# ubuntuslave/vo_single_camera_sos

Hardware: AMD Instinct MI355X
Metric: frame-pairs/sec (detect+match+triangulate+RANSAC) on 640x480 omni, 2000 kpts (higher is better)
Workload: dtype u8/f32/f64

## Files before the change

vo_single_camera_sos_amd/csrc/ransac.hip:

```cpp
#include <type_traits>
#include "common.h"
#include "ransac_core.h"
#include "epnp_core.h"
#include "gp3p_core.h"

namespace {

constexpr int kMaxCam = 8;
constexpr int kHypDoubles = 16;
constexpr int kThreads = 256;
constexpr int kScoreHypChunkMax = 128;

__device__ const double kEye9[9] = {1, 0, 0, 0, 1, 0, 0, 0, 1};
__device__ const double kZero3[3] = {0, 0, 0};

__device__ __forceinline__ uint64_t problem_seed(uint64_t seed, int b) { return seed + (uint64_t)b; }
__device__ __forceinline__ uint64_t problem_seed(const uint64_t* seeds, int b) { return seeds[b]; }

__global__ __launch_bounds__(kThreads) void ransac_prepare_kernel(const int32_t* __restrict__ cam,
                                                                  const int32_t* __restrict__ n_arr, int stride,
                                                                  int ncam, int32_t* __restrict__ perm,
                                                                  int32_t* __restrict__ cinfo) {
  SOSVO_LATENCY_BOUND_PRIO();
  __shared__ int cnt[kThreads][kMaxCam];
// ... 116 lines not shown
  const int it = chunk * 64 + threadIdx.x;
  const int n = min(n_arr[b], stride);
  const size_t base = (size_t)b * stride;
  double R[9], t[3];
  int ok = 0;
  if (it < H) ok = sv_hypothesis_twopt(f + 3 * base, p + 3 * base, n, problem_seed(seed, b), (uint64_t)it, R, t);
  hyp_store_wave(hyp + (size_t)b * H * kHypDoubles, chunk * 64, H, ok != 0, R, t);
  if (it < H) counts[(size_t)b * H + it] = ok ? 0 : -1;
}

template <class SeedT>
__global__ __launch_bounds__(64) __attribute__((amdgpu_waves_per_eu(3, 3))) void ransac_hyp_gp3p_kernel(const double* __restrict__ f, const double* __restrict__ p,
                                                             const int32_t* __restrict__ cam,
                                                             const double* __restrict__ cam_off,
                                                             const double* __restrict__ cam_rot,
                                                             const int32_t* __restrict__ n_arr, int nprob, int stride,
                                                             int H, SeedT seed, double* __restrict__ hyp,
                                                             int32_t* __restrict__ counts) {
  SOSVO_LATENCY_BOUND_PRIO();
  int b, chunk;
  if (!hyp_block(nprob, (H + 63) >> 6, &b, &chunk)) return;
  const int it = chunk * 64 + threadIdx.x;
  const int n = min(n_arr[b], stride);
  const size_t base = (size_t)b * stride;
  const double* off = cam ? cam_off : kZero3;
  const double* rot = cam ? cam_rot : kEye9;
  double R[9], t[3];
  int ok = 0;
  if (it < H)
    ok = sv_hypothesis_gp3p(f + 3 * base, p + 3 * base, cam ? cam + base : nullptr, off, rot, n, problem_seed(seed, b),
                            (uint64_t)it, R, t);
  hyp_store_wave(hyp + (size_t)b * H * kHypDoubles, chunk * 64, H, ok != 0, R, t);
  if (it < H) counts[(size_t)b * H + it] = ok ? 0 : -1;
}

__device__ __forceinline__ int epnp_sample_front(const double* __restrict__ f, const double* __restrict__ p, int n, size_t base,
                                                 uint64_t seed, int it, double (&p6)[18], double (&uv)[2 * SV_EPNP_MAXN],
                                                 double (&cw)[12], double (&alphas)[4 * SV_EPNP_MAXN]) {
  int32_t s6[6];
  if (!sv_sample_distinct(n, 6, seed, (uint64_t)it, s6)) return 0;
  double f6[18];
#pragma unroll
  for (int k = 0; k < 6; ++k)
#pragma unroll
    for (int c = 0; c < 3; ++c) {
      f6[3 * k + c] = f[3 * (base + s6[k]) + c];
      p6[3 * k + c] = p[3 * (base + s6[k]) + c];
    }
  return sv_epnp_front(f6, p6, 6, uv, cw, alphas);
}

constexpr int kEpnpVecDoubles = 48;
template <class SeedT>
__global__ __launch_bounds__(64) void ransac_epnp_eigen_kernel(const double* __restrict__ f, const double* __restrict__ p,
                                                               const int32_t* __restrict__ n_arr, int nprob, int stride,
                                                               int H, SeedT seed, double* __restrict__ vvbuf,
                                                               int32_t* __restrict__ counts) {
  int b, chunk;
  if (!hyp_block(nprob, (H + 63) >> 6, &b, &chunk)) return;
  const int it = chunk * 64 + threadIdx.x;
  if (it >= H) return;
  const int n = min(n_arr[b], stride);
  double p6[18], uv[2 * SV_EPNP_MAXN], cw[12], alphas[4 * SV_EPNP_MAXN];
  int ok = epnp_sample_front(f, p, n, (size_t)b * stride, problem_seed(seed, b), it, p6, uv, cw, alphas);
  double* out = vvbuf + ((size_t)b * H + it) * kEpnpVecDoubles;
  if (ok) {
    double vv[48];
    ok = sv_epnp_null4_ql(alphas, uv, 6, vv);
    if (ok) {
#pragma unroll
      for (int k = 0; k < 48; ++k) out[k] = vv[k];
    }
  }
  counts[(size_t)b * H + it] = ok ? 0 : -1;
}

template <class SeedT>
__global__ __launch_bounds__(64) void ransac_epnp_pose_kernel(const double* __restrict__ f, const double* __restrict__ p,
                                                              const int32_t* __restrict__ n_arr, int nprob, int stride,
                                                              int H, SeedT seed, const double* __restrict__ vvbuf,
                                                              double* __restrict__ hyp, int32_t* __restrict__ counts) {
  SOSVO_LATENCY_BOUND_PRIO();
  int b, chunk;
  if (!hyp_block(nprob, (H + 63) >> 6, &b, &chunk)) return;
  const int it = chunk * 64 + threadIdx.x;
  const int n = min(n_arr[b], stride);
  double R[9], t[3];
  int ok = it < H && counts[(size_t)b * H + it] == 0;
  if (ok) {
    double p6[18], uv[2 * SV_EPNP_MAXN], cw[12], alphas[4 * SV_EPNP_MAXN], vv[48];
    ok = epnp_sample_front(f, p, n, (size_t)b * stride, problem_seed(seed, b), it, p6, uv, cw, alphas);
    const double* in = vvbuf + ((size_t)b * H + it) * kEpnpVecDoubles;
#pragma unroll
    for (int k = 0; k < 48; ++k) vv[k] = in[k];
    if (ok) ok = sv_epnp_back(p6, 6, uv, cw, alphas, vv, R, t);
  }
  hyp_store_wave(hyp + (size_t)b * H * kHypDoubles, chunk * 64, H, ok != 0, R, t);
  if (it < H) counts[(size_t)b * H + it] = ok ? 0 : -1;
}

template <bool IDENT>
__device__ __forceinline__ bool inlier_exact(const double* __restrict__ h, const double fx, const double fy,
                                             const double fz, const double px, const double py, const double pz,
                                             const double ox, const double oy, const double oz, const double* Rc,
                                             const double thr) {
  const double vx = (((h[0] * px) + (h[3] * py)) + (h[6] * pz)) + h[12];
  const double vy = (((h[1] * px) + (h[4] * py)) + (h[7] * pz)) + h[13];
  const double vz = (((h[2] * px) + (h[5] * py)) + (h[8] * pz)) + h[14];
  const double wx = vx - ox, wy = vy - oy, wz = vz - oz;
  double ux = wx, uy = wy, uz = wz;
  if (!IDENT) {
    ux = ((Rc[0] * wx) + (Rc[3] * wy)) + (Rc[6] * wz);
    uy = ((Rc[1] * wx) + (Rc[4] * wy)) + (Rc[7] * wz);
    uz = ((Rc[2] * wx) + (Rc[5] * wy)) + (Rc[8] * wz);
  }
  const double nrm = sqrt(((ux * ux) + (uy * uy)) + (uz * uz));
  const double gx = ux / nrm, gy = uy / nrm, gz = uz / nrm;
  return (1.0 - (((fx * gx) + (fy * gy)) + (fz * gz))) < thr;
}

constexpr double kTier1K = 1048576.0;
constexpr double kTier1Eps = 5.9604644775390625e-08;
constexpr double kTier1QBand = 3.47 / kTier1K + 20.0 * kTier1Eps;
constexpr double kTier1Max = 1e9;
constexpr double kTier1E2 = (3.47 * kTier1K + 6.0) * 78.03 * kTier1Eps * kTier1Eps * (1.0 + 1e-4);

__device__ __forceinline__ float score_tier1_lane(double fx, double fy, double fz, double px, double py, double pz, double ox,
                                                  double oy, double oz) {
  const double p1 = fabs(px) + fabs(py) + fabs(pz);
  const double om = fmax(fabs(ox), fmax(fabs(oy), fabs(oz)));
  const double fn = fx * fx + fy * fy + fz * fz;
  const double l = (p1 * p1 + om * om) * (1.0 + 1e-6);
  return (fabs(fn - 1.0) <= 1e-6 && p1 <= kTier1Max && om <= kTier1Max) ? (float)l : __builtin_inff();
}

__device__ __forceinline__ void score_tier1_hyp(const double* __restrict__ h, float* __restrict__ hs) {
  double rho = 0.0;
#pragma unroll
  for (int k = 0; k < 9; ++k) {
    hs[k] = (float)h[k];
    rho = fmax(rho, fabs(h[k]));
  }
  const double im = fmax(fabs(h[9]), fmax(fabs(h[10]), fabs(h[11])));
  hs[9] = (float)h[9], hs[10] = (float)h[10], hs[11] = (float)h[11];
  const double chk = (((((((h[0] + h[1]) + h[2]) + h[3]) + h[4]) + h[5]) + h[6]) + h[7]) + h[8] + h[9] + h[10] + h[11];
  const double ea = kTier1E2 * fmax(rho * rho, 1.0) * (1.0 + 1e-6);
  const double eb = kTier1E2 * (im * im) * (1.0 + 1e-6) + 1e-24;
  const bool fin = chk == chk && rho <= kTier1Max && im <= kTier1Max;
  hs[12] = fin ? (float)ea : __builtin_nanf("");
  hs[13] = fin ? (float)eb : __builtin_nanf("");
  hs[14] = 0.0f, hs[15] = 0.0f;
}

template <bool IDENT, int PPT, bool T1>
__global__ __launch_bounds__(kThreads) __attribute__((amdgpu_waves_per_eu(T1 ? 4 : 1))) void ransac_score_kernel(
    const double* __restrict__ f, const double* __restrict__ p, const int32_t* __restrict__ cam,
    const double* __restrict__ cam_off, const double* __restrict__ cam_rot, const int32_t* __restrict__ n_arr,
    int stride, int H, int hchunk, int hspan, double thr, int fast_ok, const double* __restrict__ hyp,
    int32_t* __restrict__ counts, int set_lo, int set_hi, int hsplit, const int32_t* __restrict__ alive_idx,
    const int32_t* __restrict__ n_alive) {
  static_assert(!T1 || (IDENT && PPT <= 4), "tier 1 is written for the identity-rotation form");
  SOSVO_LATENCY_BOUND_PRIO();
  constexpr bool KEEP = !T1;
  __shared__ int lcnt[kScoreHypChunkMax];
  __shared__ double shyp[kScoreHypChunkMax][12];
  __shared__ unsigned long long sok[(kScoreHypChunkMax + 63) / 64];
  __shared__ int sidx[kScoreHypChunkMax];
  __shared__ int srec[kScoreHypChunkMax];
  __shared__ float shyp32[T1 ? kScoreHypChunkMax : 1][16];
  const int tid = threadIdx.x, b = blockIdx.z;
  const int n = min(n_arr[b], stride);
  const int Hb = alive_idx ? n_alive[b] : H;
  const int xspan = alive_idx ? (int)((blockIdx.x + blockIdx.z) % gridDim.x) : (int)blockIdx.x;
  if (xspan * hspan >= Hb) return;
  const int sbeg = set_lo, send = min((n + 63) >> 6, set_hi);
  const int nsets = send - sbeg;
  const int bcap = hsplit ? PPT : (kThreads / 64) * PPT;
  const int nb = (nsets + bcap - 1) / bcap;
  if ((int)blockIdx.y >= nb) return;
  const int spb = (nsets + nb - 1) / nb;
  const int set0 = hsplit ? sbeg + ((int)blockIdx.y * nsets) / nb : sbeg + (int)blockIdx.y * spb;
  const int set1 = hsplit ? sbeg + (((int)blockIdx.y + 1) * nsets) / nb : min(set0 + spb, send);
  const int p0 = set0 * 64;

  double fx[KEEP ? PPT : 1], fy[KEEP ? PPT : 1], fz[KEEP ? PPT : 1];
  double px[KEEP ? PPT : 1], py[KEEP ? PPT : 1], pz[KEEP ? PPT : 1];
  double ox[KEEP ? PPT : 1], oy[KEEP ? PPT : 1], oz[KEEP ? PPT : 1];
  float fxs[T1 ? PPT : 1], fys[T1 ? PPT : 1], fzs[T1 ? PPT : 1], pxs[T1 ? PPT : 1], pys[T1 ? PPT : 1], pzs[T1 ? PPT : 1];
  float oxs[T1 ? PPT : 1], oys[T1 ? PPT : 1], ozs[T1 ? PPT : 1], lerr[T1 ? PPT : 1];
  int rowi[PPT];
  double Rc[IDENT ? 1 : 9];
  const int wave = __builtin_amdgcn_readfirstlane(tid >> 6), lane = tid & 63;
  const int wslot = (wave + blockIdx.x + blockIdx.y + blockIdx.z) & (kThreads / 64 - 1);
  const int jstep = hsplit ? kThreads / 64 : 1, jbeg = hsplit ? wslot : 0;
  const size_t base = (size_t)b * stride;
  unsigned long long vmask[PPT];
  int nlive_v = 0;
#pragma unroll
  for (int r = 0; r < PPT; ++r) {
    const int set = set0 + (hsplit ? r : r * (kThreads / 64) + wslot);
    const int i0 = set * 64;
    const int i = i0 + lane;
    nlive_v += set < set1 ? 1 : 0;
    const bool valid = i < n;
    vmask[r] = __ballot(valid);
    rowi[r] = valid ? i : p0;
    const size_t row = base + rowi[r];
    const double lfx = f[3 * row + 0], lfy = f[3 * row + 1], lfz = f[3 * row + 2];
    const double lpx = p[3 * row + 0], lpy = p[3 * row + 1], lpz = p[3 * row + 2];
    const int c = cam ? cam[row] : 0;
    const double* o = cam ? cam_off + 3 * c : kZero3;
    const double lox = o[0], loy = o[1], loz = o[2];
    if (KEEP) {
      fx[r] = lfx, fy[r] = lfy, fz[r] = lfz;
      px[r] = lpx, py[r] = lpy, pz[r] = lpz;
      ox[r] = lox, oy[r] = loy, oz[r] = loz;
    }
    if (!IDENT) {
      const double* rc = cam ? cam_rot + 9 * c : kEye9;
#pragma unroll
      for (int k = 0; k < 9; ++k) Rc[k] = rc[k];
    }
    if (T1) {
      fxs[r] = (float)lfx, fys[r] = (float)lfy, fzs[r] = (float)lfz;
      pxs[r] = (float)lpx, pys[r] = (float)lpy, pzs[r] = (float)lpz;
      oxs[r] = (float)lox, oys[r] = (float)loy, ozs[r] = (float)loz;
      lerr[r] = score_tier1_lane(lfx, lfy, lfz, lpx, lpy, lpz, lox, loy, loz);
    }
  }
  const int nlive = __builtin_amdgcn_readfirstlane(nlive_v);
  const double c1 = 1.0 - thr;
  const double c2 = c1 * c1;
  const double c2hi = c2 * (1.0 + 1e-9), c2lo = c2 * (1.0 - 1e-9);
  const float c2hs = (float)((c2 + kTier1QBand) * (1.0 + 1e-6)), c2ls = (float)((c2 - kTier1QBand) * (1.0 - 1e-6));
  const int hend = min(Hb, (xspan + 1) * hspan);
  for (int h0 = xspan * hspan; h0 < hend; h0 += hchunk) {
  const int h1 = min(hend, h0 + hchunk);
  for (int k = tid; k < kScoreHypChunkMax; k += kThreads) lcnt[k] = 0;
  const int nh = h1 - h0;
  const double* hb = hyp + (size_t)b * H * kHypDoubles;
  static_assert(kScoreHypChunkMax == 128, "two words of solved-hypothesis flags");
  if (wave < 2) {
    const int hh = wave * 64 + lane;
    const int rec = hh < nh ? (alive_idx ? alive_idx[(size_t)b * H + h0 + hh] : h0 + hh) : 0;
    const double r00 = hh < nh ? hb[(size_t)rec * kHypDoubles] : 0.0;
    const unsigned long long okb = __ballot(hh < nh && r00 == r00);
    if (lane == 0) sok[wave] = okb;
    srec[hh] = rec;
  }
  __syncthreads();
  const unsigned long long ok0 = sok[0], ok1 = sok[1];
  const int nok = __builtin_amdgcn_readfirstlane(__popcll(ok0) + __popcll(ok1));
  for (int k = tid; k < nh * 12; k += kThreads) {
    const int hh = k / 12, e = k - hh * 12;
    const unsigned long long w = hh < 64 ? ok0 : ok1;
    if ((w >> (hh & 63)) & 1ULL) {
      const int pos = __popcll(w & ((1ULL << (hh & 63)) - 1ULL)) + (hh < 64 ? 0 : __popcll(ok0));
      const int rec = srec[hh];
      shyp[pos][e] = hb[(size_t)rec * kHypDoubles + (e < 9 ? e : e + 3)];
      if (e == 0) sidx[pos] = rec;
    }
  }
  __syncthreads();
  if (T1) {
    for (int pos = tid; pos < nok; pos += kThreads) score_tier1_hyp(shyp[pos], shyp32[pos]);
    __syncthreads();
  }

  auto tier2 = [&](auto nl, const int j, const unsigned long long* und1) -> int {
    constexpr int NL = decltype(nl)::value;
    int total = 0;
    const double* hp = shyp[j];
    const double r0 = hp[0], r1 = hp[1], r2 = hp[2], r3 = hp[3], r4 = hp[4], r5 = hp[5], r6 = hp[6], r7 = hp[7], r8 = hp[8];
    const double ix = hp[9], iy = hp[10], iz = hp[11];
#pragma unroll
    for (int r = 0; r < NL && r < PPT; ++r) {
      if (!und1[r]) continue;
      double Fx, Fy, Fz, Px, Py, Pz, Ox, Oy, Oz;
      if (KEEP) {
        Fx = fx[r], Fy = fy[r], Fz = fz[r], Px = px[r], Py = py[r], Pz = pz[r];
        Ox = ox[r], Oy = oy[r], Oz = oz[r];
      } else {
        const size_t row = base + rowi[r];
        Fx = f[3 * row + 0], Fy = f[3 * row + 1], Fz = f[3 * row + 2];
        Px = p[3 * row + 0], Py = p[3 * row + 1], Pz = p[3 * row + 2];
        const double* o = cam ? cam_off + 3 * cam[row] : kZero3;
        Ox = o[0], Oy = o[1], Oz = o[2];
      }
      unsigned long long und = und1[r];
      if (fast_ok) {
        double ux = fma(r0, Px, fma(r3, Py, fma(r6, Pz, ix - Ox)));
        double uy = fma(r1, Px, fma(r4, Py, fma(r7, Pz, iy - Oy)));
        double uz = fma(r2, Px, fma(r5, Py, fma(r8, Pz, iz - Oz)));
        if (!IDENT) {
          const double wx = ux, wy = uy, wz = uz;
          ux = fma(Rc[0], wx, fma(Rc[IDENT ? 0 : 3], wy, Rc[IDENT ? 0 : 6] * wz));
          uy = fma(Rc[IDENT ? 0 : 1], wx, fma(Rc[IDENT ? 0 : 4], wy, Rc[IDENT ? 0 : 7] * wz));
          uz = fma(Rc[IDENT ? 0 : 2], wx, fma(Rc[IDENT ? 0 : 5], wy, Rc[IDENT ? 0 : 8] * wz));
        }
        const double s = fma(Fx, ux, fma(Fy, uy, Fz * uz));
        const double q = fma(ux, ux, fma(uy, uy, uz * uz));
        const double lhs = s * s;
        const unsigned long long pos = __ballot(s > 0.0) & und1[r];
        const unsigned long long hi = __ballot(lhs > c2hi * q);
        const unsigned long long lo = __ballot(lhs < c2lo * q);
        total += __popcll(pos & hi);
        und = pos & ~hi & ~lo;
      }
      if (und) {
        const double vx = (((r0 * Px) + (r3 * Py)) + (r6 * Pz)) + ix;
        const double vy = (((r1 * Px) + (r4 * Py)) + (r7 * Pz)) + iy;
        const double vz = (((r2 * Px) + (r5 * Py)) + (r8 * Pz)) + iz;
        const double wx = vx - Ox, wy = vy - Oy, wz = vz - Oz;
        double ux = wx, uy = wy, uz = wz;
        if (!IDENT) {
          ux = ((Rc[0] * wx) + (Rc[IDENT ? 0 : 3] * wy)) + (Rc[IDENT ? 0 : 6] * wz);
          uy = ((Rc[IDENT ? 0 : 1] * wx) + (Rc[IDENT ? 0 : 4] * wy)) + (Rc[IDENT ? 0 : 7] * wz);
          uz = ((Rc[IDENT ? 0 : 2] * wx) + (Rc[IDENT ? 0 : 5] * wy)) + (Rc[IDENT ? 0 : 8] * wz);
        }
        const double q = ((ux * ux) + (uy * uy)) + (uz * uz);
        const double nrm = sqrt(q);
        const double gx = ux / nrm, gy = uy / nrm, gz = uz / nrm;
        total += __popcll(__ballot((1.0 - (((Fx * gx) + (Fy * gy)) + (Fz * gz))) < thr) & und);
      }
    }
    return total;
  };

  auto tier1 = [&](auto nl, const int j, unsigned long long* und1, unsigned long long& any1) -> int {
    constexpr int NL = decltype(nl)::value;
    int total = 0;
    const float* hs = shyp32[T1 ? j : 0];
    const float q0 = hs[0], q1 = hs[1], q2 = hs[2], q3 = hs[3], q4 = hs[4], q5 = hs[5], q6 = hs[6], q7 = hs[7], q8 = hs[8];
    const float jx = hs[9], jy = hs[10], jz = hs[11], ea = hs[12], eb = hs[13];
#pragma unroll
    for (int r = 0; r < NL && r < PPT; ++r) {
      const float ux = fmaf(q0, pxs[T1 ? r : 0], fmaf(q3, pys[T1 ? r : 0], fmaf(q6, pzs[T1 ? r : 0], jx - oxs[T1 ? r : 0])));
      const float uy = fmaf(q1, pxs[T1 ? r : 0], fmaf(q4, pys[T1 ? r : 0], fmaf(q7, pzs[T1 ? r : 0], jy - oys[T1 ? r : 0])));
      const float uz = fmaf(q2, pxs[T1 ? r : 0], fmaf(q5, pys[T1 ? r : 0], fmaf(q8, pzs[T1 ? r : 0], jz - ozs[T1 ? r : 0])));
      const float sv = fmaf(fxs[T1 ? r : 0], ux, fmaf(fys[T1 ? r : 0], uy, fzs[T1 ? r : 0] * uz));
      const float qv = fmaf(ux, ux, fmaf(uy, uy, uz * uz));
      const float lhs = sv * fabsf(sv);
      const float e2 = fmaf(ea, lerr[T1 ? r : 0], eb);
      const unsigned long long hi = __ballot(lhs > fmaf(c2hs, qv, e2));
      const unsigned long long lo = __ballot(lhs < fmaf(c2ls, qv, -e2));
      total += __popcll(hi & vmask[r]);
      und1[r] = ~hi & ~lo & vmask[r];
      any1 |= und1[r];
    }
    return total;
  };

  auto hyp_loop = [&](auto nl) {
    constexpr int NL = decltype(nl)::value;
    int cntv = 0, k = 0;
    for (int j = jbeg; j < nok; j += jstep, ++k) {
      unsigned long long und[PPT], any = 0ULL;
      int tot = 0;
      if (T1) {
        tot = tier1(nl, j, und, any);
      } else {
#pragma unroll
        for (int r = 0; r < NL && r < PPT; ++r) {
          und[r] = vmask[r];
          any |= vmask[r];
        }
      }
      if (any) tot += tier2(nl, j, und);
      if (lane == (k & 63)) cntv += tot;
      if ((k & 63) == 63) {
        if (cntv) atomicAdd(&lcnt[jbeg + ((k & ~63) + lane) * jstep], cntv);
        cntv = 0;
      }
    }
    if (cntv) atomicAdd(&lcnt[jbeg + (((k - 1) & ~63) + lane) * jstep], cntv);
  };
  if (nlive >= 4) hyp_loop(std::integral_constant<int, 4>{});
  else if (nlive == 3) hyp_loop(std::integral_constant<int, 3>{});
  else if (nlive == 2) hyp_loop(std::integral_constant<int, 2>{});
  else if (nlive == 1) hyp_loop(std::integral_constant<int, 1>{});
  __syncthreads();
  for (int k = tid; k < nok; k += kThreads) {
    const int v = lcnt[k];
    if (v) atomicAdd(&counts[(size_t)b * H + sidx[k]], v);
  }
  }
}

__global__ __launch_bounds__(kThreads) void ransac_prune_kernel(
    const double* __restrict__ f, const double* __restrict__ p, const int32_t* __restrict__ cam,
    const double* __restrict__ cam_off, const int32_t* __restrict__ n_arr, int stride, int H, int probe_sets, double thr,
    const double* __restrict__ hyp, const int32_t* __restrict__ counts, int32_t* __restrict__ alive_idx,
    int32_t* __restrict__ n_alive) {
  SOSVO_LATENCY_BOUND_PRIO();
  __shared__ long long red[kThreads / 64];
  __shared__ int redc[kThreads / 64];
  __shared__ int wave_off[kThreads / 64 + 1];
  const int tid = threadIdx.x, b = blockIdx.x, lane = tid & 63, wid = tid >> 6;
  const int n = min(n_arr[b], stride);
  const int32_t* cb = counts + (size_t)b * H;
  int32_t* ab = alive_idx + (size_t)b * H;
  long long best_key = -1;
  for (int it = tid; it < H; it += kThreads) {
    const int c = cb[it];
    const long long key = ((long long)c << 32) | (long long)(0x7FFFFFFF - it);
    if (c >= 0 && key > best_key) best_key = key;
  }
  for (int o = 32; o > 0; o >>= 1) {
    const long long other = __shfl_down(best_key, o);
    best_key = other > best_key ? other : best_key;
  }
  if (lane == 0) red[wid] = best_key;
  __syncthreads();
  best_key = red[0];
  for (int w = 1; w < kThreads / 64; ++w) best_key = red[w] > best_key ? red[w] : best_key;
  if (best_key < 0) {
    if (tid == 0) n_alive[b] = 0;
    return;
  }
  const int hstar = 0x7FFFFFFF - (int)(best_key & 0xFFFFFFFFLL);
  const double* hp = hyp + ((size_t)b * H + hstar) * kHypDoubles;
  const size_t base = (size_t)b * stride;
  int cnt = 0;
  for (int i = tid; i < n; i += kThreads) {
    const size_t row = base + i;
    const double* o = cam ? cam_off + 3 * cam[row] : kZero3;
    cnt += inlier_exact<true>(hp, f[3 * row], f[3 * row + 1], f[3 * row + 2], p[3 * row], p[3 * row + 1], p[3 * row + 2], o[0],
                              o[1], o[2], kEye9, thr) ? 1 : 0;
  }
  for (int o = 32; o > 0; o >>= 1) cnt += __shfl_down(cnt, o);
  if (lane == 0) redc[wid] = cnt;
  __syncthreads();
  const int L = ((redc[0] + redc[1]) + redc[2]) + redc[3];
  const int rest = n - min(n, probe_sets * 64);
  int running = 0;
  for (int it0 = 0; it0 < H; it0 += kThreads) {
    const int it = it0 + tid;
    const int c = it < H ? cb[it] : -1;
    const bool keep = c >= 0 && c + rest >= L;
    const unsigned long long bal = __ballot(keep);
    __syncthreads();
    if (lane == 0) wave_off[wid + 1] = __popcll(bal);
    __syncthreads();
    int off = running;
    for (int w = 0; w < wid; ++w) off += wave_off[w + 1];
    if (keep) ab[off + __popcll(bal & ((1ULL << lane) - 1ULL))] = it;
    running += ((wave_off[1] + wave_off[2]) + wave_off[3]) + wave_off[4];
  }
  if (tid == 0) n_alive[b] = running;
}

template <bool IDENT>
__global__ __launch_bounds__(kThreads) void ransac_select_kernel(
    const double* __restrict__ f, const double* __restrict__ p, const int32_t* __restrict__ cam,
    const double* __restrict__ cam_off, const double* __restrict__ cam_rot, const int32_t* __restrict__ n_arr,
    int stride, int H, double thr, int adaptive, const double* __restrict__ hyp, const int32_t* __restrict__ counts,
    double* __restrict__ T_out, uint8_t* __restrict__ mask, int32_t* __restrict__ inl_idx,
    int32_t* __restrict__ n_inl, int32_t* __restrict__ info) {
  SOSVO_LATENCY_BOUND_PRIO();
  __shared__ long long red[kThreads / 64];
  __shared__ int redv[kThreads / 64];
  __shared__ int s_best_it, s_used, s_nvalid;
  __shared__ int wave_off[kThreads / 64 + 1];
  __shared__ int s_running;
  const int tid = threadIdx.x, b = blockIdx.x, lane = tid & 63, wid = tid >> 6;
  const int n = min(n_arr[b], stride);
  const int32_t* cb = counts + (size_t)b * H;

  long long best_key = -1;
  int nvalid = 0;
  for (int it = tid; it < H; it += kThreads) {
    const int c = cb[it];
    if (c >= 0) {
      nvalid++;
      const long long key = ((long long)c << 32) | (long long)(0x7FFFFFFF - it);
      best_key = key > best_key ? key : best_key;
    }
  }
  for (int o = 32; o > 0; o >>= 1) {
    const long long other = __shfl_down(best_key, o);
    best_key = other > best_key ? other : best_key;
    nvalid += __shfl_down(nvalid, o);
  }
  if (lane == 0) {
    red[wid] = best_key;
    redv[wid] = nvalid;
  }
  __syncthreads();
  if (tid == 0) {
    long long k = red[0];
    int nv = redv[0];
    for (int w = 1; w < kThreads / 64; ++w) {
      k = red[w] > k ? red[w] : k;
      nv += redv[w];
    }
    s_nvalid = nv;
    if (!(adaptive & 1)) {
      s_best_it = k < 0 ? -1 : (0x7FFFFFFF - (int)(k & 0xFFFFFFFFLL));
      s_used = H;
    } else {
      int best_count = -1, best_it = -1, iterations = 0, used = 0;
      double base = 1.0;
      for (int it = 0; it < H; ++it) {
        if (iterations > 0 && !sv_ransac_continue(base, iterations)) break;
        used = it + 1;
        const int c = cb[it];
        if (c < 0) continue;
        if (c > best_count) {
          best_count = c;
          best_it = it;
          base = (adaptive & 2) ? sv_adaptive_base6(c, n) : ((adaptive & 4) ? sv_adaptive_base2(c, n) : sv_adaptive_base(c, n));
        }
        iterations++;
      }
      s_best_it = best_it;
      s_used = used;
    }
    s_running = 0;
  }
  __syncthreads();
  const int best_it = s_best_it;
  const size_t base = (size_t)b * stride;
  if (best_it < 0) {
    for (int i = tid; i < n; i += kThreads) mask[base + i] = 0;
    if (tid < 12) T_out[(size_t)b * 12 + tid] = (tid == 0 || tid == 5 || tid == 10) ? 1.0 : 0.0;
    if (tid == 0) {
      n_inl[b] = 0;
      info[4 * b + 0] = -1;
      info[4 * b + 1] = s_used;
      info[4 * b + 2] = 1;
      info[4 * b + 3] = s_nvalid;
    }
    return;
  }
  const double* hp = hyp + ((size_t)b * H + best_it) * kHypDoubles;
  for (int i0 = 0; i0 < n; i0 += kThreads) {
    const int i = i0 + tid;
    bool inl = false;
    if (i < n) {
// ... 88 lines not shown
      sv_residual_jac(x, f + 3 * row, p + 3 * row, o, rc, &r, J, Hq);
      c += r * r;
      int a = 0;
#pragma unroll
      for (int u = 0; u < 6; ++u) {
        g[u] += J[u] * r;
#pragma unroll
        for (int v = u; v < 6; ++v) {
          A[a] += (J[u] * J[v]) + Hq[a];
          a++;
        }
      }
    }
    {
      double wv[28];
      wv[27] = c;
#pragma unroll
      for (int a = 0; a < 21; ++a) wv[a] = A[a];
#pragma unroll
      for (int a = 0; a < 6; ++a) wv[21 + a] = g[a];
#pragma unroll
      for (int a = 0; a < 28; ++a)
        for (int o = 32; o > 0; o >>= 1) wv[a] = wv[a] + __shfl_down(wv[a], o);
      __syncthreads();
      if ((tid & 63) == 0) {
#pragma unroll
        for (int a = 0; a < 28; ++a) sred[a][tid >> 6] = wv[a];
      }
      __syncthreads();
      if (tid < 21) sA[tid] = ((sred[tid][0] + sred[tid][1]) + sred[tid][2]) + sred[tid][3];
      if (tid >= 21 && tid < 27) sg[tid - 21] = ((sred[tid][0] + sred[tid][1]) + sred[tid][2]) + sred[tid][3];
      cost = ((sred[27][0] + sred[27][1]) + sred[27][2]) + sred[27][3];
    }
    __syncthreads();
    int accepted = 0, converged = 0;
    for (int tries = 0; tries < SV_LM_MAX_TRIES; ++tries) {
      if (tid == 0) {
        double dx[6];
        if (sv_solve_damped(sA, sg, lambda, dx)) {
#pragma unroll
          for (int u = 0; u < 6; ++u) {
            sdx[u] = dx[u];
            sxn[u] = sx[u] + dx[u];
          }
          double dxn = 0.0, xnn = 0.0;
#pragma unroll
          for (int u = 0; u < 6; ++u) {
            dxn += dx[u] * dx[u];
            xnn += sxn[u] * sxn[u];
          }
          s_flag = (sqrt(dxn) <= SV_LM_XTOL * (sqrt(xnn) + SV_LM_XTOL)) ? 4 : 0;
        } else {
          s_flag = 3;
        }
      }
      __syncthreads();
      if (s_flag == 3) {
        lambda *= 10.0;
        __syncthreads();
        continue;
      }
      if (s_flag == 4) {
        converged = 1;
        __syncthreads();
        break;
      }
      double xn[6];
#pragma unroll
      for (int u = 0; u < 6; ++u) xn[u] = sxn[u];
      double cn = 0.0;
      for (int q = tid; q < cnt; q += kThreads) {
        const int i = idx ? idx[base + q] : q;
        const size_t row = base + i;
        const int cc = cam ? cam[row] : 0;
        const double* o = cam ? cam_off + 3 * cc : kZero3;
        const double* rc = cam ? cam_rot + 9 * cc : kEye9;
        const double r = sv_residual(xn, f + 3 * row, p + 3 * row, o, rc);
        cn += r * r;
      }
      cn = block_sum(cn, scratch, tid);
      if (cn < cost) {
        converged = ((cost - cn) <= SV_LM_FTOL * cost);
        __syncthreads();
        if (tid == 0) {
#pragma unroll
          for (int u = 0; u < 6; ++u) sx[u] = xn[u];
        }
        cost = cn;
        lambda *= 0.1;
        if (lambda < 1e-15) lambda = 1e-15;
        accepted = 1;
        __syncthreads();
        break;
      }
      lambda *= 10.0;
      __syncthreads();
    }
    it_done = it + 1;
    if (!accepted || converged) break;
  }
  __syncthreads();
  if (tid == 0) {
    double R[9], t[3];
    sv_cayley2rot(sx + 3, R);
    t[0] = sx[0];
    t[1] = sx[1];
    t[2] = sx[2];
    sv_Rt_to_T(R, t, T);
    if (cost_out) cost_out[b] = cost;
    if (iters_out) iters_out[b] = it_done;
  }
}

}

template <class SeedT>
static int32_t ransac_abs_pose_impl(sosvo_ctx* ctx, const char* fn, const double* f, const double* p, const int32_t* cam,
                                    const double* cam_off, const double* cam_rot, int32_t ncam, int32_t flags,
                                    const int32_t* n, int32_t nprob, int32_t stride, double thr, int32_t max_iter,
                                    int32_t adaptive, SeedT seed, double* T_out,
                                    uint8_t* inlier_mask, int32_t* inlier_idx, int32_t* n_inliers, int32_t* info,
                                    int32_t* hyp_counts) {
#define SOSVO_LAUNCH_HYP(ctx, kernel, ...)              \
  do {                                                  \
    SOSVO_PROFILE(ctx, #kernel);                        \
    hipLaunchKernelGGL((kernel<SeedT>), __VA_ARGS__);   \
  } while (0)
#define SOSVO_REQUIRE_FN(ctx, cond, msg)                               \
  do {                                                                 \
    if (!(cond)) return sosvo_fail((ctx), SOSVO_ERR_ARG, fn, msg);     \
  } while (0)
  SOSVO_REQUIRE_FN(ctx, f && p && n && T_out && inlier_mask && inlier_idx && n_inliers && info, "null pointer");
  SOSVO_REQUIRE_FN(ctx, cam == nullptr || (cam_off && cam_rot), "cam given without cam_off / cam_rot");
  SOSVO_REQUIRE_FN(ctx, ncam >= 1 && ncam <= kMaxCam, "ncam out of range (1..8)");
  SOSVO_REQUIRE_FN(ctx, nprob >= 0 && nprob <= 65535, "nprob out of range");
  SOSVO_REQUIRE_FN(ctx, stride > 0 && stride <= (1 << 20), "stride out of range");
  SOSVO_REQUIRE_FN(ctx, max_iter > 0 && max_iter <= (1 << 20), "max_iter out of range");
  SOSVO_REQUIRE_FN(ctx, thr > 0.0, "threshold must be positive");
  if (nprob == 0) return SOSVO_OK;
  const int H = max_iter;
  size_t off = 0;
  auto carve = [&](size_t bytes) {
    size_t o = off;
    off += (bytes + 255) & ~(size_t)255;
    return o;
  };
  const size_t o_perm = carve(sizeof(int32_t) * (size_t)nprob * stride);
  const size_t o_cinfo = carve(sizeof(int32_t) * (size_t)nprob * (2 * kMaxCam + 1));
  const size_t o_hyp = carve(sizeof(double) * (size_t)nprob * H * kHypDoubles);
  const size_t o_counts = carve(sizeof(int32_t) * (size_t)nprob * H);
  const bool epnp_vec = (flags & SOSVO_FLAG_EPNP) != 0;
  const size_t o_vv = carve(epnp_vec ? sizeof(double) * (size_t)nprob * H * kEpnpVecDoubles : 0);
  const size_t o_alive = carve(sizeof(int32_t) * (size_t)nprob * (H + 1));
  int32_t rc = sosvo_ws_reserve(ctx, off);
  if (rc != SOSVO_OK) return rc;
  char* ws = (char*)ctx->ws;
  int32_t* perm = (int32_t*)(ws + o_perm);
  int32_t* cinfo = (int32_t*)(ws + o_cinfo);
  double* hyp = (double*)(ws + o_hyp);
  int32_t* counts = hyp_counts ? hyp_counts : (int32_t*)(ws + o_counts);

  SOSVO_LAUNCH(ctx,ransac_prepare_kernel, dim3(nprob), dim3(kThreads), 0, ctx->stream, cam, n, stride,
                     cam ? ncam : 1, perm, cinfo);
  SOSVO_LAUNCH_CHECK(ctx);
  const int epnp = (flags & SOSVO_FLAG_EPNP) != 0;
  SOSVO_REQUIRE_FN(ctx, !epnp || cam == nullptr, "SOSVO_FLAG_EPNP is for central problems (cam == NULL)");
  const int twopt = (flags & SOSVO_FLAG_TWOPT) != 0 && !epnp && !(flags & SOSVO_FLAG_GP3P);
  SOSVO_REQUIRE_FN(ctx, !twopt || cam == nullptr, "SOSVO_FLAG_TWOPT is for central problems (cam == NULL)");
  if (epnp) adaptive = (adaptive ? 1 : 0) | 2;
  if (twopt) adaptive = (adaptive ? 1 : 0) | 4;
  if (epnp) {
    double* vvbuf = (double*)(ws + o_vv);
    SOSVO_LAUNCH_HYP(ctx, ransac_epnp_eigen_kernel, dim3(hyp_grid(nprob, cdiv(H, 64))), dim3(64), 0, ctx->stream, f, p, n, nprob, stride, H,
                 seed, vvbuf, counts);
    SOSVO_LAUNCH_HYP(ctx, ransac_epnp_pose_kernel, dim3(hyp_grid(nprob, cdiv(H, 64))), dim3(64), 0, ctx->stream, f, p, n, nprob, stride, H,
                 seed, vvbuf, hyp, counts);
  } else if (twopt) {
    SOSVO_LAUNCH_HYP(ctx, ransac_hyp_twopt_kernel, dim3(hyp_grid(nprob, cdiv(H, 64))), dim3(64), 0, ctx->stream, f, p, n, nprob, stride, H, seed,
                 hyp, counts);
  } else if (flags & SOSVO_FLAG_GP3P) {
    SOSVO_LAUNCH_HYP(ctx, ransac_hyp_gp3p_kernel, dim3(hyp_grid(nprob, cdiv(H, 64))), dim3(64), 0, ctx->stream, f, p, cam, cam_off, cam_rot,
                 n, nprob, stride, H, seed, hyp, counts);
  } else
    SOSVO_LAUNCH_HYP(ctx, ransac_hyp_kernel, dim3(hyp_grid(nprob, cdiv(H, 64))), dim3(64), 0, ctx->stream, f, p, cam, cam_off, cam_rot, n,
                 nprob, stride, H, seed, perm, cinfo, hyp, counts);
  SOSVO_LAUNCH_CHECK(ctx);

  const bool ident = (flags & SOSVO_FLAG_CAM_ROT_IDENTITY) != 0 || cam == nullptr;
  const int fast_ok = thr < 0.5 ? 1 : 0;
  const int ppt = ident ? 4 : 1;
  const int gx = cdiv(stride, kThreads * ppt);
  const bool t1 = ident && fast_ok && !ctx->hint_score_fp64_only;
  const int wg_target = t1 ? 4096 : 8192;
  int hchunks = cdiv(wg_target, nprob);
  if (hchunks < 1) hchunks = 1;
  int hspan = cdiv(H, hchunks);
  if (hspan < 32) hspan = H < 32 ? H : 32;
  hchunks = cdiv(H, hspan);
  const int hchunk = cdiv(hspan, cdiv(hspan, kScoreHypChunkMax));
  dim3 grid(hchunks, gx, nprob);
  constexpr int kProbeSets = 4, kPruneMinSets = 8, kPruneMinProblems = 64;
  const bool prune = t1 && adaptive == 0 && hyp_counts == nullptr && !epnp && !twopt && stride >= 64 * kPruneMinSets &&
                     nprob >= kPruneMinProblems;
#define SOSVO_SCORE_ARGS grid, dim3(kThreads), 0, ctx->stream, f, p, cam, cam_off, cam_rot, n, stride, H, hchunk, hspan, thr, fast_ok, hyp, counts, 0, INT_MAX, 0, (const int32_t*)nullptr, (const int32_t*)nullptr
  if (prune) {
    int32_t* alive_idx = (int32_t*)(ws + o_alive);
    int32_t* n_alive = alive_idx + (size_t)nprob * H;
    auto pass = [&](int set_lo, int set_hi, int hs, const int32_t* list, const int32_t* nlist) {
      const int hck = cdiv(hs, cdiv(hs, kScoreHypChunkMax));
      const int sets = min(set_hi, cdiv(stride, 64)) - set_lo;
      SOSVO_LAUNCH(ctx,(ransac_score_kernel<true, 4, true>), dim3(cdiv(H, hs), cdiv(sets, 4), nprob), dim3(kThreads), 0,
                   ctx->stream, f, p, cam, cam_off, cam_rot, n, stride, H, hck, hs, thr, fast_ok, hyp, counts, set_lo, set_hi, 1,
                   list, nlist);
    };
    pass(0, kProbeSets, min(H, 4 * hspan), nullptr, nullptr);
    SOSVO_LAUNCH(ctx,ransac_prune_kernel, dim3(nprob), dim3(kThreads), 0, ctx->stream, f, p, cam, cam_off, n, stride, H,
                 kProbeSets, thr, hyp, counts, alive_idx, n_alive);
    pass(kProbeSets, INT_MAX, min(H, max(kScoreHypChunkMax, 2 * hspan)), alive_idx, n_alive);
  } else if (t1)
    SOSVO_LAUNCH(ctx,(ransac_score_kernel<true, 4, true>), SOSVO_SCORE_ARGS);
  else if (ident)
    SOSVO_LAUNCH(ctx,(ransac_score_kernel<true, 4, false>), SOSVO_SCORE_ARGS);
  else
    SOSVO_LAUNCH(ctx,(ransac_score_kernel<false, 1, false>), SOSVO_SCORE_ARGS);
#undef SOSVO_SCORE_ARGS
  SOSVO_LAUNCH_CHECK(ctx);
  if (ident)
    SOSVO_LAUNCH(ctx,(ransac_select_kernel<true>), dim3(nprob), dim3(kThreads), 0, ctx->stream, f, p, cam,
                       cam_off, cam_rot, n, stride, H, thr, adaptive, hyp, counts, T_out, inlier_mask, inlier_idx,
                       n_inliers, info);
  else
    SOSVO_LAUNCH(ctx,(ransac_select_kernel<false>), dim3(nprob), dim3(kThreads), 0, ctx->stream, f, p, cam,
                       cam_off, cam_rot, n, stride, H, thr, adaptive, hyp, counts, T_out, inlier_mask, inlier_idx,
                       n_inliers, info);
  SOSVO_LAUNCH_CHECK(ctx);
  return SOSVO_OK;
}
#undef SOSVO_REQUIRE_FN
#undef SOSVO_LAUNCH_HYP

extern "C" {

int32_t sosvo_ransac_abs_pose(sosvo_ctx* ctx, const double* f, const double* p, const int32_t* cam,
                              const double* cam_off, const double* cam_rot, int32_t ncam, int32_t flags,
                              const int32_t* n, int32_t nprob, int32_t stride, double thr, int32_t max_iter,
                              int32_t adaptive, uint64_t seed, double* T_out, uint8_t* inlier_mask,
                              int32_t* inlier_idx, int32_t* n_inliers, int32_t* info, int32_t* hyp_counts) {
  SOSVO_ENTER(ctx);
  return ransac_abs_pose_impl(ctx, __func__, f, p, cam, cam_off, cam_rot, ncam, flags, n, nprob, stride, thr, max_iter, adaptive,
                              seed, T_out, inlier_mask, inlier_idx, n_inliers, info, hyp_counts);
}

int32_t sosvo_ransac_abs_pose_seeds(sosvo_ctx* ctx, const double* f, const double* p, const int32_t* cam,
                                    const double* cam_off, const double* cam_rot, int32_t ncam, int32_t flags,
                                    const int32_t* n, int32_t nprob, int32_t stride, double thr, int32_t max_iter,
                                    int32_t adaptive, const uint64_t* seeds, double* T_out, uint8_t* inlier_mask,
                                    int32_t* inlier_idx, int32_t* n_inliers, int32_t* info, int32_t* hyp_counts) {
  SOSVO_ENTER(ctx);
  SOSVO_REQUIRE(ctx, seeds, "null seed array");
  return ransac_abs_pose_impl(ctx, __func__, f, p, cam, cam_off, cam_rot, ncam, flags, n, nprob, stride, thr, max_iter, adaptive,
                              seeds, T_out, inlier_mask, inlier_idx, n_inliers, info, hyp_counts);
}

int32_t sosvo_refine_abs_pose(sosvo_ctx* ctx, const double* f, const double* p, const int32_t* cam,
                              const double* cam_off, const double* cam_rot, int32_t ncam, const int32_t* n,
                              int32_t nprob, int32_t stride, const int32_t* idx, const int32_t* m,
                              int32_t max_lm_iter, double* T_io, double* cost_out, int32_t* iters_out) {
  SOSVO_ENTER(ctx);
  SOSVO_REQUIRE(ctx, f && p && n && T_io, "null pointer");
  SOSVO_REQUIRE(ctx, cam == nullptr || (cam_off && cam_rot), "cam given without cam_off / cam_rot");
  SOSVO_REQUIRE(ctx, (idx == nullptr) == (m == nullptr), "idx and m go together");
  SOSVO_REQUIRE(ctx, ncam >= 1 && ncam <= kMaxCam, "ncam out of range (1..8)");
  SOSVO_REQUIRE(ctx, nprob >= 0 && nprob <= 65535, "nprob out of range");
  SOSVO_REQUIRE(ctx, stride > 0 && stride <= (1 << 20), "stride out of range");
  SOSVO_REQUIRE(ctx, max_lm_iter > 0 && max_lm_iter <= 10000, "max_lm_iter out of range");
  if (nprob == 0) return SOSVO_OK;
  SOSVO_LAUNCH(ctx,refine_kernel, dim3(nprob), dim3(kThreads), 0, ctx->stream, f, p, cam, cam_off, cam_rot, n,
                     stride, idx, m, max_lm_iter, T_io, cost_out, iters_out);
  SOSVO_LAUNCH_CHECK(ctx);
  return SOSVO_OK;
}

}
```

Baseline: 69340.

## Precompute fp32 tier-1 hypothesis records once and specialise scoring for camera-uniform waves

Adds a records kernel that converts every solved hypothesis to its fp32 tier-1 form once and compacts the solved indices. A new prepared scoring kernel loads these records with float4 reads instead of rebuilding them per block in both prune passes, and the probe pass iterates only over solved hypotheses. It also detects waves whose points all share one camera and precomputes the translation-minus-offset per hypothesis in shared memory, removing three subtractions per point per hypothesis. The cost is an extra launch and workspace, plus tier-2 reading fp64 hypotheses straight from global memory instead of shared memory.

```diff
diff --git a/vo_single_camera_sos_amd/csrc/ransac.hip b/vo_single_camera_sos_amd/csrc/ransac.hip
--- a/vo_single_camera_sos_amd/csrc/ransac.hip
+++ b/vo_single_camera_sos_amd/csrc/ransac.hip
@@ -292,22 +292,26 @@
   hs[14] = 0.0f, hs[15] = 0.0f;
 }
 
-template <bool IDENT, int PPT, bool T1>
-__global__ __launch_bounds__(kThreads) __attribute__((amdgpu_waves_per_eu(T1 ? 4 : 1))) void ransac_score_kernel(
+template <bool IDENT, int PPT, bool T1, bool PREP>
+__device__ __forceinline__ void ransac_score_body(
     const double* __restrict__ f, const double* __restrict__ p, const int32_t* __restrict__ cam,
     const double* __restrict__ cam_off, const double* __restrict__ cam_rot, const int32_t* __restrict__ n_arr,
     int stride, int H, int hchunk, int hspan, double thr, int fast_ok, const double* __restrict__ hyp,
     int32_t* __restrict__ counts, int set_lo, int set_hi, int hsplit, const int32_t* __restrict__ alive_idx,
-    const int32_t* __restrict__ n_alive) {
+    const int32_t* __restrict__ n_alive, const float* __restrict__ rec32) {
   static_assert(!T1 || (IDENT && PPT <= 4), "tier 1 is written for the identity-rotation form");
+  static_assert(!PREP || T1, "prepared records are tier-1 records");
   SOSVO_LATENCY_BOUND_PRIO();
   constexpr bool KEEP = !T1;
+  constexpr int kNW = kThreads / 64;
   __shared__ int lcnt[kScoreHypChunkMax];
-  __shared__ double shyp[kScoreHypChunkMax][12];
+  __shared__ double shyp[PREP ? 1 : kScoreHypChunkMax][12];
   __shared__ unsigned long long sok[(kScoreHypChunkMax + 63) / 64];
   __shared__ int sidx[kScoreHypChunkMax];
-  __shared__ int srec[kScoreHypChunkMax];
-  __shared__ float shyp32[T1 ? kScoreHypChunkMax : 1][16];
+  __shared__ int srec[PREP ? 1 : kScoreHypChunkMax];
+  __shared__ __attribute__((aligned(16))) float shyp32[T1 ? kScoreHypChunkMax : 1][16];
+  __shared__ __attribute__((aligned(16))) float sdc[T1 ? 2 : 1][T1 ? kScoreHypChunkMax : 1][4];
+  __shared__ int swcam[kNW];
   const int tid = threadIdx.x, b = blockIdx.z;
   const int n = min(n_arr[b], stride);
   const int Hb = alive_idx ? n_alive[b] : H;
@@ -336,6 +340,8 @@
   const size_t base = (size_t)b * stride;
   unsigned long long vmask[PPT];
   int nlive_v = 0;
+  int wcam = -1;
+  bool wuni = true;
 #pragma unroll
   for (int r = 0; r < PPT; ++r) {
     const int set = set0 + (hsplit ? r : r * (kThreads / 64) + wslot);
@@ -349,6 +355,11 @@
     const double lfx = f[3 * row + 0], lfy = f[3 * row + 1], lfz = f[3 * row + 2];
     const double lpx = p[3 * row + 0], lpy = p[3 * row + 1], lpz = p[3 * row + 2];
     const int c = cam ? cam[row] : 0;
+    if (T1 && set < set1) {
+      const int c0 = __builtin_amdgcn_readfirstlane(c);
+      if (c0 < 0 || __ballot(valid && c != c0) != 0ULL || (wcam >= 0 && wcam != c0)) wuni = false;
+      wcam = c0;
+    }
     const double* o = cam ? cam_off + 3 * c : kZero3;
     const double lox = o[0], loy = o[1], loz = o[2];
     if (KEEP) {
@@ -369,6 +380,19 @@
     }
   }
   const int nlive = __builtin_amdgcn_readfirstlane(nlive_v);
+  int wsel = -1, ca = -1, cb = -1;
+  if (T1) {
+    if (lane == 0) swcam[wave] = (nlive > 0 && wuni) ? wcam : -1;
+    __syncthreads();
+#pragma unroll
+    for (int w = 0; w < kNW; ++w) {
+      const int c = __builtin_amdgcn_readfirstlane(swcam[w]);
+      if (c >= 0 && ca < 0) ca = c;
+      else if (c >= 0 && c != ca && cb < 0) cb = c;
+    }
+    const int cw = __builtin_amdgcn_readfirstlane(swcam[wave]);
+    wsel = cw < 0 ? -1 : (cw == ca ? 0 : (cw == cb ? 1 : -1));
+  }
   const double c1 = 1.0 - thr;
   const double c2 = c1 * c1;
   const double c2hi = c2 * (1.0 + 1e-9), c2lo = c2 * (1.0 - 1e-9);
@@ -380,6 +404,33 @@
   const int nh = h1 - h0;
   const double* hb = hyp + (size_t)b * H * kHypDoubles;
   static_assert(kScoreHypChunkMax == 128, "two words of solved-hypothesis flags");
+  int nok_v;
+  float oa[3] = {0.0f, 0.0f, 0.0f}, ob[3] = {0.0f, 0.0f, 0.0f};
+  if (T1) {
+    int cal = ca, cbl = cb;
+    asm volatile("" : "+s"(cal), "+s"(cbl));
+    const double* pa = (cam && cal >= 0) ? cam_off + 3 * cal : kZero3;
+    const double* pb = (cam && cbl >= 0) ? cam_off + 3 * cbl : kZero3;
+    oa[0] = (float)pa[0], oa[1] = (float)pa[1], oa[2] = (float)pa[2];
+    ob[0] = (float)pb[0], ob[1] = (float)pb[1], ob[2] = (float)pb[2];
+  }
+  if (PREP) {
+    const int32_t* list = alive_idx + (size_t)b * H + h0;
+    const float4* rb = reinterpret_cast<const float4*>(rec32) + (size_t)b * H * 4;
+    for (int k = tid; k < nh * 4; k += kThreads) {
+      const int hh = k >> 2, q = k & 3;
+      const int rec = list[hh];
+      const float4 v = rb[(size_t)rec * 4 + q];
+      reinterpret_cast<float4*>(shyp32[T1 ? hh : 0])[q] = v;
+      if (q == 2) {
+        *reinterpret_cast<float4*>(sdc[0][T1 ? hh : 0]) = make_float4(v.y - oa[0], v.z - oa[1], v.w - oa[2], 0.0f);
+        *reinterpret_cast<float4*>(sdc[T1 ? 1 : 0][T1 ? hh : 0]) = make_float4(v.y - ob[0], v.z - ob[1], v.w - ob[2], 0.0f);
+      }
+      if (q == 3) sidx[hh] = rec;
+    }
+    nok_v = nh;
+    __syncthreads();
+  } else {
   if (wave < 2) {
     const int hh = wave * 64 + lane;
     const int rec = hh < nh ? (alive_idx ? alive_idx[(size_t)b * H + h0 + hh] : h0 + hh) : 0;
@@ -390,7 +441,7 @@
   }
   __syncthreads();
   const unsigned long long ok0 = sok[0], ok1 = sok[1];
-  const int nok = __builtin_amdgcn_readfirstlane(__popcll(ok0) + __popcll(ok1));
+  nok_v = __popcll(ok0) + __popcll(ok1);
   for (int k = tid; k < nh * 12; k += kThreads) {
     const int hh = k / 12, e = k - hh * 12;
     const unsigned long long w = hh < 64 ? ok0 : ok1;
@@ -403,16 +454,26 @@
   }
   __syncthreads();
   if (T1) {
-    for (int pos = tid; pos < nok; pos += kThreads) score_tier1_hyp(shyp[pos], shyp32[pos]);
+    for (int pos = tid; pos < nok_v; pos += kThreads) {
+      float* hs = shyp32[pos];
+      score_tier1_hyp(shyp[PREP ? 0 : pos], hs);
+      float* da = sdc[0][pos];
+      float* db = sdc[T1 ? 1 : 0][pos];
+      da[0] = hs[9] - oa[0], da[1] = hs[10] - oa[1], da[2] = hs[11] - oa[2];
+      db[0] = hs[9] - ob[0], db[1] = hs[10] - ob[1], db[2] = hs[11] - ob[2];
+    }
     __syncthreads();
   }
+  }
+  const int nok = __builtin_amdgcn_readfirstlane(nok_v);
 
   auto tier2 = [&](auto nl, const int j, const unsigned long long* und1) -> int {
     constexpr int NL = decltype(nl)::value;
     int total = 0;
-    const double* hp = shyp[j];
+    const double* hp = PREP ? hb + (size_t)sidx[j] * kHypDoubles : shyp[PREP ? 0 : j];
+    constexpr int IO = PREP ? 12 : 9;
     const double r0 = hp[0], r1 = hp[1], r2 = hp[2], r3 = hp[3], r4 = hp[4], r5 = hp[5], r6 = hp[6], r7 = hp[7], r8 = hp[8];
-    const double ix = hp[9], iy = hp[10], iz = hp[11];
+    const double ix = hp[IO], iy = hp[IO + 1], iz = hp[IO + 2];
 #pragma unroll
     for (int r = 0; r < NL && r < PPT; ++r) {
       if (!und1[r]) continue;
@@ -467,17 +528,20 @@
     return total;
   };
 
-  auto tier1 = [&](auto nl, const int j, unsigned long long* und1, unsigned long long& any1) -> int {
+  auto tier1 = [&](auto nl, auto uni, const int j, unsigned long long* und1, unsigned long long& any1) -> int {
     constexpr int NL = decltype(nl)::value;
+    constexpr bool UNI = decltype(uni)::value;
     int total = 0;
     const float* hs = shyp32[T1 ? j : 0];
     const float q0 = hs[0], q1 = hs[1], q2 = hs[2], q3 = hs[3], q4 = hs[4], q5 = hs[5], q6 = hs[6], q7 = hs[7], q8 = hs[8];
-    const float jx = hs[9], jy = hs[10], jz = hs[11], ea = hs[12], eb = hs[13];
+    const float* jd = UNI ? sdc[T1 ? wsel : 0][T1 ? j : 0] : hs + 9;
+    const float jx = jd[0], jy = jd[1], jz = jd[2], ea = hs[12], eb = hs[13];
 #pragma unroll
     for (int r = 0; r < NL && r < PPT; ++r) {
-      const float ux = fmaf(q0, pxs[T1 ? r : 0], fmaf(q3, pys[T1 ? r : 0], fmaf(q6, pzs[T1 ? r : 0], jx - oxs[T1 ? r : 0])));
-      const float uy = fmaf(q1, pxs[T1 ? r : 0], fmaf(q4, pys[T1 ? r : 0], fmaf(q7, pzs[T1 ? r : 0], jy - oys[T1 ? r : 0])));
-      const float uz = fmaf(q2, pxs[T1 ? r : 0], fmaf(q5, pys[T1 ? r : 0], fmaf(q8, pzs[T1 ? r : 0], jz - ozs[T1 ? r : 0])));
+      const float dx = UNI ? jx : jx - oxs[T1 ? r : 0], dy = UNI ? jy : jy - oys[T1 ? r : 0], dz = UNI ? jz : jz - ozs[T1 ? r : 0];
+      const float ux = fmaf(q0, pxs[T1 ? r : 0], fmaf(q3, pys[T1 ? r : 0], fmaf(q6, pzs[T1 ? r : 0], dx)));
+      const float uy = fmaf(q1, pxs[T1 ? r : 0], fmaf(q4, pys[T1 ? r : 0], fmaf(q7, pzs[T1 ? r : 0], dy)));
+      const float uz = fmaf(q2, pxs[T1 ? r : 0], fmaf(q5, pys[T1 ? r : 0], fmaf(q8, pzs[T1 ? r : 0], dz)));
       const float sv = fmaf(fxs[T1 ? r : 0], ux, fmaf(fys[T1 ? r : 0], uy, fzs[T1 ? r : 0] * uz));
       const float qv = fmaf(ux, ux, fmaf(uy, uy, uz * uz));
       const float lhs = sv * fabsf(sv);
@@ -491,14 +555,14 @@
     return total;
   };
 
-  auto hyp_loop = [&](auto nl) {
+  auto hyp_loop = [&](auto nl, auto uni) {
     constexpr int NL = decltype(nl)::value;
     int cntv = 0, k = 0;
     for (int j = jbeg; j < nok; j += jstep, ++k) {
       unsigned long long und[PPT], any = 0ULL;
       int tot = 0;
       if (T1) {
-        tot = tier1(nl, j, und, any);
+        tot = tier1(nl, uni, j, und, any);
       } else {
 #pragma unroll
         for (int r = 0; r < NL && r < PPT; ++r) {
@@ -515,16 +579,81 @@
     }
     if (cntv) atomicAdd(&lcnt[jbeg + (((k - 1) & ~63) + lane) * jstep], cntv);
   };
-  if (nlive >= 4) hyp_loop(std::integral_constant<int, 4>{});
-  else if (nlive == 3) hyp_loop(std::integral_constant<int, 3>{});
-  else if (nlive == 2) hyp_loop(std::integral_constant<int, 2>{});
-  else if (nlive == 1) hyp_loop(std::integral_constant<int, 1>{});
+  auto hyp_loops = [&](auto uni) {
+    if (nlive >= 4) hyp_loop(std::integral_constant<int, 4>{}, uni);
+    else if (nlive == 3) hyp_loop(std::integral_constant<int, 3>{}, uni);
+    else if (nlive == 2) hyp_loop(std::integral_constant<int, 2>{}, uni);
+    else if (nlive == 1) hyp_loop(std::integral_constant<int, 1>{}, uni);
+  };
+  if constexpr (T1) {
+    if (wsel >= 0) hyp_loops(std::true_type{});
+    else hyp_loops(std::false_type{});
+  } else
+    hyp_loops(std::false_type{});
   __syncthreads();
   for (int k = tid; k < nok; k += kThreads) {
     const int v = lcnt[k];
     if (v) atomicAdd(&counts[(size_t)b * H + sidx[k]], v);
   }
-  }
+  if (PREP) __syncthreads();
+  }
+}
+
+template <bool IDENT, int PPT, bool T1>
+__global__ __launch_bounds__(kThreads) __attribute__((amdgpu_waves_per_eu(T1 ? 4 : 1))) void ransac_score_kernel(
+    const double* __restrict__ f, const double* __restrict__ p, const int32_t* __restrict__ cam,
+    const double* __restrict__ cam_off, const double* __restrict__ cam_rot, const int32_t* __restrict__ n_arr,
+    int stride, int H, int hchunk, int hspan, double thr, int fast_ok, const double* __restrict__ hyp,
+    int32_t* __restrict__ counts, int set_lo, int set_hi, int hsplit, const int32_t* __restrict__ alive_idx,
+    const int32_t* __restrict__ n_alive) {
+  ransac_score_body<IDENT, PPT, T1, false>(f, p, cam, cam_off, cam_rot, n_arr, stride, H, hchunk, hspan, thr, fast_ok, hyp, counts,
+                                           set_lo, set_hi, hsplit, alive_idx, n_alive, nullptr);
+}
+
+__global__ __launch_bounds__(kThreads) __attribute__((amdgpu_waves_per_eu(4))) void ransac_score_kernel_prepared(
+    const double* __restrict__ f, const double* __restrict__ p, const int32_t* __restrict__ cam,
+    const double* __restrict__ cam_off, const int32_t* __restrict__ n_arr, int stride, int H, int hchunk, int hspan, double thr,
+    int fast_ok, const double* __restrict__ hyp, int32_t* __restrict__ counts, int set_lo, int set_hi,
+    const int32_t* __restrict__ list, const int32_t* __restrict__ nlist, const float* __restrict__ rec32) {
+  ransac_score_body<true, 4, true, true>(f, p, cam, cam_off, nullptr, n_arr, stride, H, hchunk, hspan, thr, fast_ok, hyp, counts,
+                                         set_lo, set_hi, 1, list, nlist, rec32);
+}
+
+__global__ __launch_bounds__(kThreads) void ransac_records_kernel(const double* __restrict__ hyp, int H,
+                                                                  float* __restrict__ rec32, int32_t* __restrict__ solved_idx,
+                                                                  int32_t* __restrict__ n_solved) {
+  SOSVO_LATENCY_BOUND_PRIO();
+  __shared__ int wave_off[kThreads / 64 + 1];
+  const int tid = threadIdx.x, b = blockIdx.x, lane = tid & 63, wid = tid >> 6;
+  int32_t* sb = solved_idx + (size_t)b * H;
+  int running = 0;
+  for (int it0 = 0; it0 < H; it0 += kThreads) {
+    const int it = it0 + tid;
+    bool ok = false;
+    if (it < H) {
+      const double* hp = hyp + ((size_t)b * H + it) * kHypDoubles;
+      double h[12];
+#pragma unroll
+      for (int e = 0; e < 12; ++e) h[e] = hp[e < 9 ? e : e + 3];
+      ok = h[0] == h[0];
+      if (ok) {
+        float hs[16];
+        score_tier1_hyp(h, hs);
+        float4* out = reinterpret_cast<float4*>(rec32) + ((size_t)b * H + it) * 4;
+#pragma unroll
+        for (int q = 0; q < 4; ++q) out[q] = make_float4(hs[4 * q], hs[4 * q + 1], hs[4 * q + 2], hs[4 * q + 3]);
+      }
+    }
+    const unsigned long long bal = __ballot(ok);
+    __syncthreads();
+    if (lane == 0) wave_off[wid + 1] = __popcll(bal);
+    __syncthreads();
+    int off = running;
+    for (int w = 0; w < wid; ++w) off += wave_off[w + 1];
+    if (ok) sb[off + __popcll(bal & ((1ULL << lane) - 1ULL))] = it;
+    running += ((wave_off[1] + wave_off[2]) + wave_off[3]) + wave_off[4];
+  }
+  if (tid == 0) n_solved[b] = running;
 }
 
 __global__ __launch_bounds__(kThreads) void ransac_prune_kernel(
@@ -919,6 +1048,13 @@
   const bool epnp_vec = (flags & SOSVO_FLAG_EPNP) != 0;
   const size_t o_vv = carve(epnp_vec ? sizeof(double) * (size_t)nprob * H * kEpnpVecDoubles : 0);
   const size_t o_alive = carve(sizeof(int32_t) * (size_t)nprob * (H + 1));
+  constexpr int kProbeSets = 4, kPruneMinSets = 8, kPruneMinProblems = 64;
+  const bool prune = ((flags & SOSVO_FLAG_CAM_ROT_IDENTITY) != 0 || cam == nullptr) && thr < 0.5 && !ctx->hint_score_fp64_only &&
+                     adaptive == 0 && hyp_counts == nullptr && !epnp_vec &&
+                     ((flags & SOSVO_FLAG_TWOPT) == 0 || (flags & SOSVO_FLAG_GP3P) != 0) && stride >= 64 * kPruneMinSets &&
+                     nprob >= kPruneMinProblems;
+  const size_t o_rec32 = carve(prune ? sizeof(float) * (size_t)nprob * H * 16 : 0);
+  const size_t o_solved = carve(prune ? sizeof(int32_t) * (size_t)nprob * (H + 1) : 0);
   int32_t rc = sosvo_ws_reserve(ctx, off);
   if (rc != SOSVO_OK) return rc;
   char* ws = (char*)ctx->ws;
@@ -966,21 +1102,22 @@
   hchunks = cdiv(H, hspan);
   const int hchunk = cdiv(hspan, cdiv(hspan, kScoreHypChunkMax));
   dim3 grid(hchunks, gx, nprob);
-  constexpr int kProbeSets = 4, kPruneMinSets = 8, kPruneMinProblems = 64;
-  const bool prune = t1 && adaptive == 0 && hyp_counts == nullptr && !epnp && !twopt && stride >= 64 * kPruneMinSets &&
-                     nprob >= kPruneMinProblems;
 #define SOSVO_SCORE_ARGS grid, dim3(kThreads), 0, ctx->stream, f, p, cam, cam_off, cam_rot, n, stride, H, hchunk, hspan, thr, fast_ok, hyp, counts, 0, INT_MAX, 0, (const int32_t*)nullptr, (const int32_t*)nullptr
   if (prune) {
     int32_t* alive_idx = (int32_t*)(ws + o_alive);
     int32_t* n_alive = alive_idx + (size_t)nprob * H;
+    float* rec32 = (float*)(ws + o_rec32);
+    int32_t* solved_idx = (int32_t*)(ws + o_solved);
+    int32_t* n_solved = solved_idx + (size_t)nprob * H;
+    SOSVO_LAUNCH(ctx,ransac_records_kernel, dim3(nprob), dim3(kThreads), 0, ctx->stream, hyp, H, rec32, solved_idx, n_solved);
     auto pass = [&](int set_lo, int set_hi, int hs, const int32_t* list, const int32_t* nlist) {
       const int hck = cdiv(hs, cdiv(hs, kScoreHypChunkMax));
       const int sets = min(set_hi, cdiv(stride, 64)) - set_lo;
-      SOSVO_LAUNCH(ctx,(ransac_score_kernel<true, 4, true>), dim3(cdiv(H, hs), cdiv(sets, 4), nprob), dim3(kThreads), 0,
-                   ctx->stream, f, p, cam, cam_off, cam_rot, n, stride, H, hck, hs, thr, fast_ok, hyp, counts, set_lo, set_hi, 1,
-                   list, nlist);
+      SOSVO_LAUNCH(ctx,ransac_score_kernel_prepared, dim3(cdiv(H, hs), cdiv(sets, 4), nprob), dim3(kThreads), 0,
+                   ctx->stream, f, p, cam, cam_off, n, stride, H, hck, hs, thr, fast_ok, hyp, counts, set_lo, set_hi, list, nlist,
+                   rec32);
     };
-    pass(0, kProbeSets, min(H, 4 * hspan), nullptr, nullptr);
+    pass(0, kProbeSets, min(H, 4 * hspan), solved_idx, n_solved);
     SOSVO_LAUNCH(ctx,ransac_prune_kernel, dim3(nprob), dim3(kThreads), 0, ctx->stream, f, p, cam, cam_off, n, stride, H,
                  kProbeSets, thr, hyp, counts, alive_idx, n_alive);
     pass(kProbeSets, INT_MAX, min(H, max(kScoreHypChunkMax, 2 * hspan)), alive_idx, n_alive);
```

After: 69900 (median of 6 runs). About the same (+0.8%).
